# zamazincode/cv-diffusion-model

Measured on AMD Instinct MI355X. Metric: images/sec (whole node), 256×256 4-step LCM 'small'; PSNR vs CPU ref, higher is better.
Workload: dtype fp16; 1 GPU; variant=small, 256x256, batch=32/GPU, 4 LCM steps, fp16, 1xMI355X (BASELINE configs[1] per GPU); global_batch=32, parallelism=single GPU

## Files before the change

cv-diffusion-model_amd/_native.py:

```python
from __future__ import annotations

import ctypes as C
import os
from typing import List, Tuple

_HERE = os.path.dirname(os.path.abspath(__file__))
LIB_PATH = os.path.join(_HERE, "libllie_hip.so")

LLIE_F32, LLIE_F16, LLIE_BF16 = 0, 1, 2
LLIE_UNET, LLIE_IRB, LLIE_ATTN, LLIE_DOWN, LLIE_UP, LLIE_SE = 0, 1, 2, 3, 4, 5
ERR_ARG, ERR_SHAPE, ERR_CONFIG, ERR_KEY, ERR_NOT_LOADED, ERR_WORKSPACE, ERR_NO_DEVICE = -1, -2, -3, -4, -5, -6, -7

EXPORTS = [
    "llie_last_error", "llie_version", "llie_create", "llie_destroy", "llie_num_params", "llie_param_info",
    "llie_load_param", "llie_params_loaded", "llie_workspace_bytes", "llie_unet_forward", "llie_module_forward",
    "llie_lcm_step", "llie_add_noise", "llie_enhance", "llie_algorithmic_bytes", "llie_flops",
    "llie_profile_begin", "llie_profile_end", "llie_enhance_workspace_bytes",
    "llie_preprocess_u8", "llie_postprocess_u8", "llie_profile_report", "llie_pw_gemm", "llie_pw_gemm_tile_rows", "llie_dwconv3x3", "llie_dwconv3x3_tiles", "llie_tune",
    "llie_grad_numel", "llie_param_grad_offset", "llie_train_workspace_bytes", "llie_unet_train_forward",
    "llie_unet_backward", "llie_module_backward", "llie_load_all", "llie_profile_dump", "llie_copy_probe", "llie_rw_probe", "llie_pw_expand", "llie_gram_stats", "llie_gram_part_floats", "llie_groupnorm_finalize", "llie_conv3x3", "llie_conv3x3_tiles", "llie_linattn", "llie_linattn_splits", "llie_se_mlp", "llie_film", "llie_refresh_params", "llie_path_bytes", "llie_time_embed", "llie_debug_irbx_stamps", "llie_debug_gemm_stamps", "llie_debug_pwx_stamps", "llie_graph_cache_entries", "llie_debug_conv_stamps", "llie_gram_finalize",
    "llie_optimizer_create", "llie_optimizer_destroy", "llie_optimizer_numel", "llie_optimizer_step",
    "llie_optimizer_step_amp",
    "llie_consistency_target", "llie_consistency_loss", "llie_ema_create", "llie_ema_update", "llie_ema_destroy",
    "llie_wgrad", "llie_wgrad_msplit", "llie_wgrad_partial_floats", "llie_dw_wgrad", "llie_dw_wgrad_strips",
    "llie_groupnorm_backward", "llie_groupnorm_backward_scratch_floats", "llie_linattn_backward", "llie_linattn_dkv_floats",
    "llie_upsample2x_backward", "llie_dilate2x", "llie_linear_dx", "llie_linear_dx_scratch_floats", "llie_linear_dw",
    "llie_final_bwd_data",
    "llie_dwconv3x3_backward", "llie_groupnorm_backward_from_slab", "llie_bias_grad", "llie_bias_grad_floats", "llie_pack_planes",
    "llie_add_into", "llie_sin_embed", "llie_pointwise_backward",
    "llie_tile_count", "llie_tile_origins", "llie_tile_gather_u8", "llie_tile_gather_f32", "llie_tile_blend_u8",
    "llie_aug_pair_u8", "llie_aug_synth_u8",
    "llie_image_metrics_scratch_bytes", "llie_image_metrics_f32", "llie_image_metrics_u8", "llie_comparison_grid_u8",
    "llie_upconv_fold_elems", "llie_upconv_fold_weights", "llie_conv3x3_upfold", "llie_conv3x3_upfold_tiles",
    "llie_expand_dw", "llie_expand_pool", "llie_expand_dw_project", "llie_expand_dw_project_skip", "llie_irbx_project_tiles",
    "llie_expand_stats", "llie_irbx_stats_rows",
    "llie_dwconv3x3_ex", "llie_dwconv3x3_strip_rows", "llie_last_kernel",
    "llie_init_conv", "llie_init_conv_tiles", "llie_init_conv_pack_bytes", "llie_final_conv", "llie_final_conv_pack_bytes",
    "llie_se_gate", "llie_affine_add", "llie_nchw_to_nhwc", "llie_nhwc_to_nchw", "llie_pw_gemm_dot",
    "llie_frame_shape_ok", "llie_frame_workspace_bytes", "llie_unet_forward_hw", "llie_enhance_hw",
    "llie_frame_pad", "llie_frame_load_u8", "llie_frame_store_u8",
]
K_GEMM, K_DW, K_CONV3, K_SE, K_OTHER = 1, 2, 4, 8, 16
PW_SIGMOID_BWD, PW_RELU6_BWD, PW_SILU_BWD, PW_SCALE = 0, 1, 2, 3


class GemmSeg(C.Structure):
    _fields_ = [("ptr", C.c_void_p), ("channels", C.c_int), ("scale", C.c_void_p), ("bias", C.c_void_p),
                ("affine_ld", C.c_int), ("act", C.c_int)]


# ... 143 lines not shown
    L.llie_init_conv_pack_bytes.restype = i64
    L.llie_init_conv_tiles.argtypes = [ci, ci, ci]
    L.llie_init_conv.argtypes = [ci, vp, ci, vp, ci, vp, vp, vp, vp, ci, ci, ci, ci, ci, vp, i64, vp]
    L.llie_final_conv_pack_bytes.argtypes = [ci]
    L.llie_final_conv_pack_bytes.restype = i64
    L.llie_final_conv.argtypes = [ci, vp, vp, vp, vp, vp, vp, ci, ci, ci, ci, ci, ci, C.POINTER(StepCoef), vp, vp, vp, vp, vp, i64, vp]
    L.llie_se_gate.argtypes = [ci, vp, ci, vp, vp, vp, vp, vp, ci, ci, ci, ci, vp, vp, vp]
    L.llie_affine_add.argtypes = [ci, vp, vp, vp, vp, vp, vp, ci, ci, ci, vp]
    L.llie_nchw_to_nhwc.argtypes = [ci, vp, vp, vp, ci, ci, ci, ci, ci, vp]
    L.llie_nhwc_to_nchw.argtypes = [ci, vp, vp, ci, ci, ci, ci, ci, vp]
    L.llie_pw_gemm_dot.argtypes = [ci, C.POINTER(GemmSeg), ci, vp, vp, vp, vp, vp, ci, ci, ci, vp]
    L.llie_last_kernel.argtypes = []
    L.llie_last_kernel.restype = C.c_char_p
    L.llie_expand_dw.argtypes = [ci, vp, ci, vp, ci, vp, vp, vp, vp, vp, vp, vp, vp, ci, ci, ci, vp]
    L.llie_expand_pool.argtypes = [ci, vp, ci, vp, ci, vp, vp, vp, vp, vp, vp, vp, ci, ci, ci, vp]
    L.llie_expand_dw_project.argtypes = [ci, vp, ci, vp, vp, vp, vp, vp, vp, vp, vp, vp, vp, ci, ci, ci, vp]
    L.llie_expand_dw_project_skip.argtypes = [ci, vp, ci, vp, ci, vp, vp, vp, vp, vp, vp, vp, vp, ci, ci, vp, vp, ci, ci, ci, vp]
    L.llie_irbx_project_tiles.argtypes = [ci, ci]
    L.llie_expand_stats.argtypes = [ci, vp, ci, vp, ci, vp, vp, vp, vp, ci, ci, ci, vp]
    L.llie_irbx_stats_rows.argtypes = [ci]
    L.llie_tune.argtypes = [C.c_char_p, ci]
    L.llie_debug_irbx_stamps.argtypes = [C.POINTER(C.c_double)]
    L.llie_optimizer_create.argtypes = [C.POINTER(OptTensor), ci, C.POINTER(C.c_void_p)]
    L.llie_optimizer_destroy.argtypes = [C.c_void_p]
    L.llie_optimizer_destroy.restype = None
    L.llie_optimizer_numel.argtypes = [C.c_void_p]
    L.llie_optimizer_numel.restype = C.c_int64
    L.llie_optimizer_step.argtypes = [C.c_void_p, vp, C.POINTER(OptHyper), vp, vp]
    L.llie_optimizer_step_amp.argtypes = [C.c_void_p, vp, C.POINTER(OptHyper), C.POINTER(AmpState), C.POINTER(AmpConfig), vp, vp]
    L.llie_consistency_target.argtypes = [vp, vp, vp, vp, vp, ci, vp, ci, i64, vp]
# ... 192 lines not shown
```

cv-diffusion-model_amd/csrc/common.h:

```cpp
#pragma once
#include <hip/hip_runtime.h>
#include <stdint.h>

#include <atomic>
#include <type_traits>

#include "kernels.h"

namespace llie {

typedef _Float16 half_t;
typedef __bf16 bf16_t;

typedef float f32x4 __attribute__((ext_vector_type(4)));
typedef float f32x16 __attribute__((ext_vector_type(16)));
typedef _Float16 f16x8 __attribute__((ext_vector_type(8)));
typedef _Float16 f16x2 __attribute__((ext_vector_type(2)));
typedef __bf16 bf16x8 __attribute__((ext_vector_type(8)));
typedef uint32_t u32x4 __attribute__((ext_vector_type(4)));
typedef f32x4 f32x4u __attribute__((aligned(4)));

constexpr int kWave = 64;

__device__ __forceinline__ void load12(const uint8_t* s, uint32_t (&b)[12]) {
// ... 117 lines not shown
  if constexpr (std::is_same<T, half_t>::value) {
    uint32_t r;
    if constexpr (CLAMP) {
      asm("v_fma_mixlo_f16 %0, %1, %2, %3 op_sel:[0,0,0] op_sel_hi:[1,0,0] clamp" : "=v"(r) : "v"(x2), "v"(s0), "v"(b0));
      asm("v_fma_mixhi_f16 %0, %1, %2, %3 op_sel:[1,0,0] op_sel_hi:[1,0,0] clamp" : "+v"(r) : "v"(x2), "v"(s1), "v"(b1));
    } else {
      asm("v_fma_mixlo_f16 %0, %1, %2, %3 op_sel:[0,0,0] op_sel_hi:[1,0,0]" : "=v"(r) : "v"(x2), "v"(s0), "v"(b0));
      asm("v_fma_mixhi_f16 %0, %1, %2, %3 op_sel:[1,0,0] op_sel_hi:[1,0,0]" : "+v"(r) : "v"(x2), "v"(s1), "v"(b1));
    }
    return r;
  } else {
    return affine_clamp01_pack<T, CLAMP>(__uint_as_float(x2 << 16), __uint_as_float(x2 & 0xFFFF0000u), s0, s1, b0, b1);
  }
}

__device__ __forceinline__ float wave_sum(float v) {
#pragma unroll
  for (int o = 32; o > 0; o >>= 1) v += __shfl_xor(v, o, 64);
  return v;
}
__device__ __forceinline__ double wave_sum(double v) {
#pragma unroll
  for (int o = 32; o > 0; o >>= 1) v += __shfl_xor(v, o, 64);
  return v;
}

constexpr int kPoolSegRows = 8;
template <int VEC>
__device__ __forceinline__ void pool_segment_flush(float (&psum)[VEC], float* red_wave , int lane) {
  static_assert(VEC == 8 || VEC == 4, "");
// ... 89 lines not shown
```

cv-diffusion-model_amd/csrc/engine.h:

```cpp
#pragma once
#include <hip/hip_runtime.h>

#include <algorithm>
#include <cmath>
#include <cstdarg>
#include <cstdio>
#include <cstdlib>
#include <cstring>
#include <map>
#include <tuple>
#include <string>
#include <vector>

#include "../../include/llie.h"
#include "kernels.h"

namespace llie {

void set_err(const char* fmt, ...);
inline hipStream_t hs(llie_stream stream) { return reinterpret_cast<hipStream_t>(stream); }

inline size_t elem_size(int dt) { return dt == LLIE_F32 ? 4 : 2; }
inline size_t align_up(size_t x, size_t a) { return (x + a - 1) / a * a; }

// ... 178 lines not shown
    if (hipEventCreate(&e) != hipSuccess) return nullptr;
    return e;
  }
};

namespace llie {

struct Knobs {
  int use_irbx;
  int irbx_project;
  int gram;
  int nt_min_mb;
  int nt_mask;
  int se_mfma;
  int bwd_async;
  int upconv_fold;
  int enhance_split;
  int epoch;
};
extern Knobs g_knobs;

enum IrbForm { kIrbUnfused, kIrbRecompute, kIrbProject };
struct IrbPath {
  IrbForm form;
  bool s6;
  bool fixtot;
  bool gram;
};
inline IrbPath irb_path(int dt, const IrbW& w, int c0, int H, int W, bool training) {
  IrbPath p{kIrbUnfused, !training && dt != LLIE_F32, !training && w.hid % 128 == 0, false};
  if (!p.fixtot || !g_knobs.use_irbx || w.hid != w.hid_r || w.cin != w.cin_r || !irbx_supported(dt, w.cin, c0, w.hid, H, W)) return p;
  p.gram = g_knobs.gram && (H * W >= 32768 || g_knobs.gram > 1) && gram_supported(dt, w.cin, c0, H * W);
  const int tail = g_knobs.irbx_project && w.cout == w.cout_r ? irbx_project_supported(dt, w.cin, c0, w.hid, w.cout, w.skip, H, W) : 0;
  p.form = tail && !(tail == kIrbxProjectSkip && g_knobs.irbx_project == 2) ? kIrbProject : kIrbRecompute;
  return p;
}

inline bool upconv_fold_supported(int dt, int Hi, int Wi, int C) {
  return g_knobs.upconv_fold && (C == 64 || C == 128) && conv3x3_upfold_ok(dt, Hi, Wi, C);
}

struct Exec {
  llie_ctx* c;
  Arena* ar;
  hipStream_t s;
// ... 40 lines not shown
```

cv-diffusion-model_amd/csrc/forward.cpp:

```cpp
#include "engine.h"

using namespace llie;

namespace {

struct Run : Exec {
  Tape* tape = nullptr;
  char tag[56] = "";
  void rel(size_t off) { if (!tape) ar->free(off); }
  size_t zoff = 0, zcur = 0, zcap = 0;
  bool zcount = false;
  template <typename F> void zbegin(int H, int W, F&& forward_again) {
    if (tape || zcount) return;
    const auto key = std::make_tuple(B, H, W, g_knobs.epoch);
    auto it = c->zneed.find(key);
    if (it == c->zneed.end()) {
      size_t zbytes = 0;
      plan(c, B, forward_again, &zbytes);
      it = c->zneed.emplace(key, zbytes).first;
    }
    zcap = it->second;
    if (!zcap) return;
    zoff = ar->alloc(zcap);
    if (!dry) chk(launch_zero_fill(ws + zoff, (int64_t)zcap, s));
// ... 115 lines not shown
    gn(h1, nullptr, w.n2g, w.n2b, film, film_stride, t.as2, t.ab2, &rec.n2, path.s6 ? 1.f / 6.f : 0.f);
    t.dnt = dwconv_ntiles(H, W);
    t.h2 = ar->alloc((size_t)M * w.hid * es());
    t.pool = path.fixtot ? 0 : ar->alloc((size_t)B * t.dnt * w.hid * 4);
    t.ptot = path.fixtot ? ztake((size_t)B * w.hid * 8) : 0;
    if (!dry) {
      DwArgs d{};
      d.in = p(h1.off); d.out = p(t.h2); d.as = p<float>(t.as2); d.ab = p<float>(t.ab2); d.w = wptr<float>(w.w_dw);
      if (path.fixtot) d.pool_tot = p<unsigned long long>(t.ptot); else d.pool = p<float>(t.pool);
      d.B = B; d.H = H; d.W = W; d.C = w.hid; d.s6 = path.s6 ? 1 : 0; d.nt = nt_store(4, (int64_t)M * w.hid);
      timed(LLIE_K_DW, 2LL * M * w.hid * (int64_t)es(), [&] { return launch_dwconv3x3(dt, d, s); });
    }
    rel(t.as1); rel(t.ab1); rel(h1.off); rel(h1.slab); rel(t.as2); rel(t.ab2);
  }

  IrbxArgs irbx_args(const IrbW& w, const Tens& x0, const Tens* x1, size_t as1, size_t ab1) const {
    IrbxArgs a{};
    a.x0 = p(x0.off); a.c0 = x0.C; a.x1 = x1 ? p(x1->off) : nullptr; a.c1 = x1 ? x1->C : 0; a.as1 = p<float>(as1); a.ab1 = p<float>(ab1);
    a.w1 = wptr(w.w_expand); a.wd = wptr<float>(w.w_dw); a.B = B; a.H = x0.H; a.W = x0.W; a.Chid = w.hid;
    return a;
  }
  void front_recompute(const IrbPath& path, const IrbW& w, const Tens& x0, const Tens* x1, const float* film, int64_t film_stride, IrbTmp& t) {
    const int H = x0.H, W = x0.W, P = H * W, M = B * P;
    const bool pool_only = path.form == kIrbProject;
    Tens st;
    st.C = w.hid; st.Cr = w.hid_r; st.H = H; st.W = W; st.ntiles = P / irbx_stats_rows(P); st.valid = true;
    st.slab = path.gram ? 0 : ar->alloc((size_t)B * st.ntiles * 2 * w.hid * 4);
    const size_t gpart = path.gram ? ar->alloc((size_t)B * gram_part_floats(w.cin, P) * 4) : 0;
    const size_t gtot = path.gram ? ar->alloc((size_t)B * (w.cin * w.cin + w.cin) * 4) : 0;
    const size_t gtick = path.gram ? ztake((size_t)B * 4) : 0;
// ... 96 lines not shown
            [&] { return launch_expand_dw_project(dt, a, w.cout, w.skip, s); });
    }
    rel(t.as1); rel(t.ab1); rel(t.as2); rel(t.ab2); rel(t.gate);
    return y;
  }

  Tens irb(const IrbW& w, const Tens& x0, const Tens* x1, const float* film, int64_t film_stride) {
    const int P = x0.H * x0.W;
    const IrbPath path = irb_path(dt, w, x0.C, x0.H, x0.W, tape != nullptr);
    IrbRec rec{};
    IrbTmp t;
    snprintf(tag, sizeof tag, "irb P=%d %d->%d hid=%d", P, w.cin, w.cout, w.hid);
    gn(x0, x1, w.n1g, w.n1b, nullptr, 0, t.as1, t.ab1, &rec.n1, path.s6 ? 1.f / 6.f : 0.f);
    const float* film2 = film ? film + w.film_off : nullptr;
    if (path.form == kIrbUnfused) front_unfused(path, w, x0, x1, film2, film_stride, rec, t);
    else front_recompute(path, w, x0, x1, film2, film_stride, t);
    se_gate(path, w, P, t);
    Tens y = path.form == kIrbProject ? project_fused(w, x0, t) : project_gemm(w, x0, x1, t);
    if (tape) {
      rec.w = (int)(&w - c->irbs.data());
      rec.x0 = x0; rec.cat = x1 != nullptr;
      if (x1) rec.x1 = *x1;
      rec.h1 = t.h1; rec.h2 = t.h2; rec.gate = t.gate; rec.sehid = t.sehid; rec.semean = t.semean; rec.y = y;
      tape->ops.push_back({0, (int)tape->irbs.size()});
      tape->irbs.push_back(rec);
    }
    return y;
  }

  Tens attn(const AttnW& w, const Tens& x) {
// ... 339 lines not shown
```

cv-diffusion-model_amd/csrc/irbx.hip:

```cpp
#include <string>
#include <type_traits>
#include <vector>

#include "common.h"
#include "kernels.h"

namespace llie {

typedef uint32_t u32x2 __attribute__((ext_vector_type(2)));

typedef __bf16 bf16x2_t __attribute__((ext_vector_type(2)));
__device__ __forceinline__ float dot2_bf16(uint32_t a, uint32_t b, float c) {
  return __builtin_amdgcn_fdot2_f32_bf16(*reinterpret_cast<const bf16x2_t*>(&a), *reinterpret_cast<const bf16x2_t*>(&b), c, false);
}

template <typename T>
__device__ __forceinline__ typename Elem<T>::vec_t activate8(typename Elem<T>::vec_t v, const float* sc, const float* sh) {
  const u32x4 x = reinterpret_cast<const u32x4&>(v);
  const f32x4 s0 = *reinterpret_cast<const f32x4*>(sc), s1 = *reinterpret_cast<const f32x4*>(sc + 4);
  const f32x4 b0 = *reinterpret_cast<const f32x4*>(sh), b1 = *reinterpret_cast<const f32x4*>(sh + 4);
  u32x4 o;
  o[0] = act_clamp01_pack<T>(x[0], s0[0], s0[1], b0[0], b0[1]);
  o[1] = act_clamp01_pack<T>(x[1], s0[2], s0[3], b0[2], b0[3]);
  o[2] = act_clamp01_pack<T>(x[2], s1[0], s1[1], b1[0], b1[1]);
  o[3] = act_clamp01_pack<T>(x[3], s1[2], s1[3], b1[2], b1[3]);
  return reinterpret_cast<const typename Elem<T>::vec_t&>(o);
}

constexpr int kXStamps = 9;
template <typename T> struct PackedOne;
template <> struct PackedOne<half_t> { static constexpr uint32_t lo = 0x00003C00u, hi = 0x3C000000u; };
template <> struct PackedOne<bf16_t> { static constexpr uint32_t lo = 0x00003F80u, hi = 0x3F800000u; };
template <typename T> __device__ __forceinline__ float dot2_pk(uint32_t a, uint32_t b, float c) {
  if constexpr (std::is_same<T, half_t>::value)
    return __builtin_amdgcn_fdot2(*reinterpret_cast<const f16x2*>(&a), *reinterpret_cast<const f16x2*>(&b), c, false);
  else return dot2_bf16(a, b, c);
}

template <typename T, int KS, int NBW, bool POOL, bool STAMP = false>
__device__ __forceinline__ void expand_scan(const IrbxArgs& a, const int RP) {
  constexpr int K = 16 * KS, XP = (K + 8) * 2;
// ... 938 lines not shown
```

cv-diffusion-model_amd/csrc/kernel_api.cpp:

```cpp
#include "engine.h"

using namespace llie;

static bool dtype_ok(int dtype) { return dtype >= 0 && dtype <= 2; }

int llie::kerr(const char* what, hipError_t e, int refuse_rc, const char* refuse_msg) {
  if (e == hipSuccess) return LLIE_OK;
  if (e == hipErrorInvalidValue && refuse_rc) {
    if (refuse_msg) set_err("%s: %s", what, refuse_msg);
    return refuse_rc;
  }
  set_err("%s: %s", what, hipGetErrorString(e));
  return (int)e;
}

static int to_segs(const llie_gemm_seg* segs, int nseg, GemmSeg* out) {
  int K = 0;
  for (int i = 0; i < nseg; ++i) {
    out[i] = GemmSeg{segs[i].ptr, segs[i].channels, segs[i].scale, segs[i].bias, segs[i].affine_ld, segs[i].act};
    K += segs[i].channels;
  }
  return K;
}

// ... 740 lines not shown
  a.gate = gate; a.wp = w_project; a.y = y; a.ystats = stats;
  return kerr("expand_dw_project", launch_expand_dw_project(dtype, a, C, false, hs(stream)), LLIE_ERR_SHAPE,
              "2-byte dtype, C in {32, 64}, H % 8 == 0, W % 16 == 0");
}
int llie_expand_dw_project_skip(int dtype, const void* x0, int c0, const void* x1, int c1, const float* scale1, const float* shift1,
                                const void* w_expand, const float* scale2, const float* shift2, const float* w_dw, const float* gate,
                                const void* w_project_skip, int ld, int cout, void* y, float* stats, int batch, int H, int W, llie_stream stream) {
  if (!x0 || !scale1 || !shift1 || !w_expand || !scale2 || !shift2 || !w_dw || !gate || !w_project_skip || !y || !stats || batch <= 0 || c0 <= 0 ||
      c1 < 0 || (c1 > 0) != (x1 != nullptr) || cout <= 0 || ld < 5 * (c0 + c1))
    return LLIE_ERR_ARG;
  IrbxArgs a = irbx_args(x0, c0, x1, c1, scale1, shift1, w_expand, scale2, shift2, w_dw, batch, H, W);
  a.gate = gate; a.wp = w_project_skip; a.ldp = ld; a.y = y; a.ystats = stats;
  return kerr("expand_dw_project_skip", launch_expand_dw_project(dtype, a, cout, true, hs(stream)), LLIE_ERR_SHAPE,
              "2-byte dtype, c0 + c1 == 96, c0 % 16 == 0, cout == 32, ld % 8 == 0, H % 8 == 0, W % 16 == 0");
}
int llie_irbx_project_tiles(int H, int W) { return H > 0 && W > 0 && H % 8 == 0 && W % 16 == 0 ? irbx_project_tiles(H, W) : LLIE_ERR_ARG; }

int llie_dwconv3x3_tiles(int H, int W) { return dwconv_ntiles(H, W); }
int llie_pw_gemm_tile_rows(int P) { return pw_gemm_tile_rows(P); }
}
```

cv-diffusion-model_amd/csrc/kernels.h:

```cpp
#pragma once
#include <hip/hip_runtime.h>
#include <stdint.h>

namespace llie {

enum Act : int { ACT_NONE = 0, ACT_RELU6 = 1, ACT_SILU = 2, ACT_RELU6_S6 = 3 };

void note_kernel(const char* name);
const char* last_kernel();

struct StatSrc {
  const float* slab;
  int ntiles;
  int ch;
};

struct GemmSeg {
  const void* ptr;
  int ch;
  const float* as;
  const float* ab;
  int aff_ld;
  int act;
};
// ... 118 lines not shown
};
void irbx_grid(int ks, int v);
void irbx_stamp(int v);
hipError_t irbx_stamp_fetch(double* out10);
bool irbx_supported(int dtype, int Cin, int c0, int Chid, int H, int W);
int irbx_pool_tiles(int H, int W);
constexpr int kIrbxProjectIdentity = 1, kIrbxProjectSkip = 2;
int irbx_project_supported(int dtype, int Cin, int c0, int Chid, int Cout, bool skip, int H, int W);
int irbx_project_tiles(int H, int W);
int irbx_stats_rows(int P);
void irbx_tune(int dbuf);
hipError_t launch_expand_stats(int dtype, const IrbxArgs& a, hipStream_t s);
hipError_t launch_expand_dw(int dtype, const IrbxArgs& a, hipStream_t s);
hipError_t launch_expand_pool(int dtype, const IrbxArgs& a, hipStream_t s);
hipError_t launch_expand_dw_project(int dtype, const IrbxArgs& a, int cout, bool skip, hipStream_t s);
int dwconv_ntiles(int H, int W);
int dw_pick_tyl(int B, int H, int W, int chunks);

struct SeArgs {
  const float* pool; int ntiles; int P;
  int pool_stride;
  const void* w1; const float* b1;
  const void* w2; const float* b2;
  float* mean;
  float* hid;
  float* gate;
  int B, C, Cs;
  const unsigned long long* tot;
  long long* pre;
};
// ... 330 lines not shown
```

cv-diffusion-model_amd/csrc/tune.cpp:

```cpp
#include "engine.h"

using namespace llie;

static Knobs knob_defaults() {
  Knobs k{};
  k.use_irbx = getenv("LLIE_NO_IRBX") ? 0 : 1;
  k.irbx_project = 1;
  k.gram = 1;
  k.nt_min_mb = 100; k.nt_mask = 1;
  k.upconv_fold = 1;
  k.se_mfma = 1;
  k.bwd_async = 1;
  k.enhance_split = getenv("LLIE_ENHANCE_SPLIT") ? atoi(getenv("LLIE_ENHANCE_SPLIT")) : 2;
  k.epoch = 0;
  return k;
}
Knobs llie::g_knobs = knob_defaults();

static hipError_t elapsed_ms(const llie_ctx::ProfRec& r, float* ms) {
  hipError_t e = hipEventSynchronize(r.e1);
  if (e == hipSuccess) e = hipEventElapsedTime(ms, r.e0, r.e1);
  if (e != hipSuccess) set_err("profile: %s", hipGetErrorString(e));
  return e;
}

// ... 2 lines not shown
  hipError_t e = hipDeviceSynchronize();
  if (e == hipSuccess) e = fetch(out);
  return e == hipSuccess ? LLIE_OK : LLIE_ERR_ARG;
}

extern "C" {

int llie_tune(const char* knob, int value) {
  if (!knob) return LLIE_ERR_ARG;
  ++g_knobs.epoch;
  if (!strcmp(knob, "gemm_bk")) { pw_gemm_force_bk(value); return LLIE_OK; }
  if (!strcmp(knob, "se_mfma")) { g_knobs.se_mfma = value; return LLIE_OK; }
  if (!strcmp(knob, "nt_min_mb")) { g_knobs.nt_min_mb = value; return LLIE_OK; }
  if (!strcmp(knob, "nt_mask")) { g_knobs.nt_mask = value; return LLIE_OK; }
  if (!strcmp(knob, "upconv_fold")) { g_knobs.upconv_fold = value != 0; return LLIE_OK; }
  if (!strcmp(knob, "gram")) { g_knobs.gram = value; return LLIE_OK; }
  if (!strcmp(knob, "irbx")) { g_knobs.use_irbx = value != 0; return LLIE_OK; }
  if (!strcmp(knob, "irbx_project")) { g_knobs.irbx_project = value < 0 || value > 2 ? 1 : value; return LLIE_OK; }
  if (!strcmp(knob, "irbx_dbuf")) { irbx_tune(value); return LLIE_OK; }
  if (!strcmp(knob, "irbx_stamp")) { irbx_stamp(value); return LLIE_OK; }
  if (!strcmp(knob, "irbx_grid")) { irbx_grid(0, value); return LLIE_OK; }
  if (!strcmp(knob, "irbx_grid2")) { irbx_grid(2, value); return LLIE_OK; }
  if (!strcmp(knob, "irbx_grid4")) { irbx_grid(4, value); return LLIE_OK; }
  if (!strcmp(knob, "irbx_grid6")) { irbx_grid(6, value); return LLIE_OK; }
  if (!strcmp(knob, "conv_stamp")) { conv3x3_stamp(value); return LLIE_OK; }
  if (!strcmp(knob, "gemm_stamp")) { pw_gemm_stamp(value); return LLIE_OK; }
  if (!strcmp(knob, "pwx")) { pw_expand_enable(value); return LLIE_OK; }
  if (!strcmp(knob, "pwx_stamp")) { pw_expand_debug(value); return LLIE_OK; }
  if (!strcmp(knob, "bwd_async")) { g_knobs.bwd_async = value; return LLIE_OK; }
  if (!strcmp(knob, "enhance_split")) { g_knobs.enhance_split = value; return LLIE_OK; }
// ... 73 lines not shown
```

include/llie.h:

```cpp
#ifndef LLIE_H_
#define LLIE_H_

#include <stddef.h>
#include <stdint.h>

#ifdef __cplusplus
extern "C" {
#endif

typedef struct llie_ctx llie_ctx;
typedef void* llie_stream;

enum llie_status {
  LLIE_OK = 0,
  LLIE_ERR_ARG = -1,
  LLIE_ERR_SHAPE = -2,
  LLIE_ERR_CONFIG = -3,
  LLIE_ERR_KEY = -4,
  LLIE_ERR_NOT_LOADED = -5,
  LLIE_ERR_WORKSPACE = -6,
  LLIE_ERR_NO_DEVICE = -7
};

enum llie_dtype { LLIE_F32 = 0, LLIE_F16 = 1, LLIE_BF16 = 2 };
// ... 271 lines not shown
                   const float* scale2, const float* shift2, const float* w_dw, void* h2, unsigned long long* pool_totals, int batch, int H, int W,
                   llie_stream stream);
int llie_expand_pool(int dtype, const void* x0, int c0, const void* x1, int c1, const float* scale1, const float* shift1, const void* w_expand,
                     const float* scale2, const float* shift2, const float* w_dw, unsigned long long* pool_totals, int batch, int H, int W,
                     llie_stream stream);
int llie_expand_dw_project(int dtype, const void* x, int C, const float* scale1, const float* shift1, const void* w_expand, const float* scale2,
                           const float* shift2, const float* w_dw, const float* gate, const void* w_project, void* y, float* stats, int batch,
                           int H, int W, llie_stream stream);
int llie_expand_dw_project_skip(int dtype, const void* x0, int c0, const void* x1, int c1, const float* scale1, const float* shift1,
                                const void* w_expand, const float* scale2, const float* shift2, const float* w_dw, const float* gate,
                                const void* w_project_skip, int ld, int cout, void* y, float* stats, int batch, int H, int W, llie_stream stream);
int llie_irbx_project_tiles(int H, int W);
int llie_expand_stats(int dtype, const void* x0, int c0, const void* x1, int c1, const float* scale1, const float* shift1, const void* w_expand,
                      float* stats, int batch, int H, int W, llie_stream stream);
int llie_irbx_stats_rows(int P);
int llie_copy_probe(const void* src, void* dst, int64_t bytes, llie_stream stream);
int llie_rw_probe(const void* src, void* dst, int64_t units, int reads, int writes, int nontemporal, llie_stream stream);
int llie_tune(const char* knob, int value);
int llie_debug_irbx_stamps(double* out10);
int llie_debug_conv_stamps(double* out8);
int llie_debug_gemm_stamps(double* out3);
int llie_debug_pwx_stamps(double* out4);

enum llie_kernel_class {
  LLIE_K_GEMM = 1,
  LLIE_K_DW = 2,
  LLIE_K_CONV3 = 4,
  LLIE_K_SE = 8,
  LLIE_K_OTHER = 16
};
// ... 17 lines not shown
```

Baseline: 1207 images/sec.

## Add fused expand+groupnorm+dwconv kernel holding the whole 32x32 map in LDS

Adds a new IRB front-end kernel for 1024-pixel maps (32x32) with 128 input channels. One workgroup keeps a 64-channel slab of the expanded activations for a whole image in LDS. It runs the expand GEMM with MFMA, computes GroupNorm statistics in place, applies norm+FiLM+ReLU6, then the 3x3 depthwise conv, and writes pooled SE sums, all without writing the intermediate to HBM or launching a separate stats pass. The path is enabled by default through a knob. The cost is one workgroup per CU from about 141KB of LDS, and it applies only to low-resolution layers.

Result: no change. 1205 images/sec (-0.2%).

```diff
diff --git a/cv-diffusion-model_amd/_native.py b/cv-diffusion-model_amd/_native.py
--- a/cv-diffusion-model_amd/_native.py
+++ b/cv-diffusion-model_amd/_native.py
@@ -33,7 +33,7 @@
     "llie_image_metrics_scratch_bytes", "llie_image_metrics_f32", "llie_image_metrics_u8", "llie_comparison_grid_u8",
     "llie_upconv_fold_elems", "llie_upconv_fold_weights", "llie_conv3x3_upfold", "llie_conv3x3_upfold_tiles",
     "llie_expand_dw", "llie_expand_pool", "llie_expand_dw_project", "llie_expand_dw_project_skip", "llie_irbx_project_tiles",
-    "llie_expand_stats", "llie_irbx_stats_rows",
+    "llie_expand_stats", "llie_irbx_stats_rows", "llie_expand_dw_map", "llie_irb_map_supported",
     "llie_dwconv3x3_ex", "llie_dwconv3x3_strip_rows", "llie_last_kernel",
     "llie_init_conv", "llie_init_conv_tiles", "llie_init_conv_pack_bytes", "llie_final_conv", "llie_final_conv_pack_bytes",
     "llie_se_gate", "llie_affine_add", "llie_nchw_to_nhwc", "llie_nhwc_to_nchw", "llie_pw_gemm_dot",
@@ -207,6 +207,8 @@
     L.llie_last_kernel.restype = C.c_char_p
     L.llie_expand_dw.argtypes = [ci, vp, ci, vp, ci, vp, vp, vp, vp, vp, vp, vp, vp, ci, ci, ci, vp]
     L.llie_expand_pool.argtypes = [ci, vp, ci, vp, ci, vp, vp, vp, vp, vp, vp, vp, ci, ci, ci, vp]
+    L.llie_expand_dw_map.argtypes = [ci, vp, ci, vp, ci, vp, vp, vp, vp, vp, vp, vp, i64, C.c_float, vp, vp, vp, ci, ci, ci, vp]
+    L.llie_irb_map_supported.argtypes = [ci, ci, ci, ci, ci]
     L.llie_expand_dw_project.argtypes = [ci, vp, ci, vp, vp, vp, vp, vp, vp, vp, vp, vp, vp, ci, ci, ci, vp]
     L.llie_expand_dw_project_skip.argtypes = [ci, vp, ci, vp, ci, vp, vp, vp, vp, vp, vp, vp, vp, ci, ci, vp, vp, ci, ci, ci, vp]
     L.llie_irbx_project_tiles.argtypes = [ci, ci]
diff --git a/cv-diffusion-model_amd/csrc/common.h b/cv-diffusion-model_amd/csrc/common.h
--- a/cv-diffusion-model_amd/csrc/common.h
+++ b/cv-diffusion-model_amd/csrc/common.h
@@ -155,6 +155,19 @@
   }
 }
 
+template <typename T>
+__device__ __forceinline__ typename Elem<T>::vec_t activate8(typename Elem<T>::vec_t v, const float* sc, const float* sh) {
+  const u32x4 x = reinterpret_cast<const u32x4&>(v);
+  const f32x4 s0 = *reinterpret_cast<const f32x4*>(sc), s1 = *reinterpret_cast<const f32x4*>(sc + 4);
+  const f32x4 b0 = *reinterpret_cast<const f32x4*>(sh), b1 = *reinterpret_cast<const f32x4*>(sh + 4);
+  u32x4 o;
+  o[0] = act_clamp01_pack<T>(x[0], s0[0], s0[1], b0[0], b0[1]);
+  o[1] = act_clamp01_pack<T>(x[1], s0[2], s0[3], b0[2], b0[3]);
+  o[2] = act_clamp01_pack<T>(x[2], s1[0], s1[1], b1[0], b1[1]);
+  o[3] = act_clamp01_pack<T>(x[3], s1[2], s1[3], b1[2], b1[3]);
+  return reinterpret_cast<const typename Elem<T>::vec_t&>(o);
+}
+
 __device__ __forceinline__ float wave_sum(float v) {
 #pragma unroll
   for (int o = 32; o > 0; o >>= 1) v += __shfl_xor(v, o, 64);
diff --git a/cv-diffusion-model_amd/csrc/engine.h b/cv-diffusion-model_amd/csrc/engine.h
--- a/cv-diffusion-model_amd/csrc/engine.h
+++ b/cv-diffusion-model_amd/csrc/engine.h
@@ -216,13 +216,14 @@
   int nt_mask;
   int se_mfma;
   int bwd_async;
+  int irb_map;
   int upconv_fold;
   int enhance_split;
   int epoch;
 };
 extern Knobs g_knobs;
 
-enum IrbForm { kIrbUnfused, kIrbRecompute, kIrbProject };
+enum IrbForm { kIrbUnfused, kIrbRecompute, kIrbProject, kIrbMap };
 struct IrbPath {
   IrbForm form;
   bool s6;
@@ -231,6 +232,10 @@
 };
 inline IrbPath irb_path(int dt, const IrbW& w, int c0, int H, int W, bool training) {
   IrbPath p{kIrbUnfused, !training && dt != LLIE_F32, !training && w.hid % 128 == 0, false};
+  if (p.fixtot && p.s6 && g_knobs.irb_map && w.cin == 128 && w.has_wf && w.hid == w.hid_r && w.cin == w.cin_r && irb_map_supported(dt, w.cin, c0, w.hid, H, W)) {
+    p.form = kIrbMap;
+    return p;
+  }
   if (!p.fixtot || !g_knobs.use_irbx || w.hid != w.hid_r || w.cin != w.cin_r || !irbx_supported(dt, w.cin, c0, w.hid, H, W)) return p;
   p.gram = g_knobs.gram && (H * W >= 32768 || g_knobs.gram > 1) && gram_supported(dt, w.cin, c0, H * W);
   const int tail = g_knobs.irbx_project && w.cout == w.cout_r ? irbx_project_supported(dt, w.cin, c0, w.hid, w.cout, w.skip, H, W) : 0;
diff --git a/cv-diffusion-model_amd/csrc/forward.cpp b/cv-diffusion-model_amd/csrc/forward.cpp
--- a/cv-diffusion-model_amd/csrc/forward.cpp
+++ b/cv-diffusion-model_amd/csrc/forward.cpp
@@ -153,6 +153,22 @@
     rel(t.as1); rel(t.ab1); rel(h1.off); rel(h1.slab); rel(t.as2); rel(t.ab2);
   }
 
+  void front_map(const IrbW& w, const Tens& x0, const Tens* x1, const float* film, int64_t film_stride, IrbTmp& t) {
+    const int H = x0.H, W = x0.W, P = H * W, M = B * P;
+    t.dnt = dwconv_ntiles(H, W);
+    t.h2 = ar->alloc((size_t)M * w.hid * es());
+    t.ptot = ztake((size_t)B * w.hid * 8);
+    if (!dry) {
+      IrbMapArgs a{};
+      a.x0 = p(x0.off); a.c0 = x0.C; a.x1 = x1 ? p(x1->off) : nullptr; a.c1 = x1 ? x1->C : 0; a.as1 = p<float>(t.as1); a.ab1 = p<float>(t.ab1);
+      a.wf = wptr(w.w_expand_f); a.gamma = wptr<float>(w.n2g); a.beta = wptr<float>(w.n2b); a.film = film; a.film_stride = film_stride;
+      a.eps = 1e-5f; a.wd = wptr<float>(w.w_dw); a.out = p(t.h2); a.pool_tot = p<unsigned long long>(t.ptot);
+      a.B = B; a.H = H; a.W = W; a.Chid = w.hid;
+      timed(LLIE_K_DW, ((int64_t)M * (w.cin + w.hid) + (int64_t)w.hid * w.cin) * (int64_t)es(), [&] { return launch_expand_dw_map(dt, a, s); });
+    }
+    rel(t.as1); rel(t.ab1);
+  }
+
   IrbxArgs irbx_args(const IrbW& w, const Tens& x0, const Tens* x1, size_t as1, size_t ab1) const {
     IrbxArgs a{};
     a.x0 = p(x0.off); a.c0 = x0.C; a.x1 = x1 ? p(x1->off) : nullptr; a.c1 = x1 ? x1->C : 0; a.as1 = p<float>(as1); a.ab1 = p<float>(ab1);
@@ -279,6 +295,7 @@
     gn(x0, x1, w.n1g, w.n1b, nullptr, 0, t.as1, t.ab1, &rec.n1, path.s6 ? 1.f / 6.f : 0.f);
     const float* film2 = film ? film + w.film_off : nullptr;
     if (path.form == kIrbUnfused) front_unfused(path, w, x0, x1, film2, film_stride, rec, t);
+    else if (path.form == kIrbMap) front_map(w, x0, x1, film2, film_stride, t);
     else front_recompute(path, w, x0, x1, film2, film_stride, t);
     se_gate(path, w, P, t);
     Tens y = path.form == kIrbProject ? project_fused(w, x0, t) : project_gemm(w, x0, x1, t);
diff --git a/cv-diffusion-model_amd/csrc/irbm.hip b/cv-diffusion-model_amd/csrc/irbm.hip
--- /dev/null
+++ b/cv-diffusion-model_amd/csrc/irbm.hip
@@ -0,0 +1,284 @@
+#include <string>
+#include <type_traits>
+
+#include "common.h"
+#include "kernels.h"
+
+namespace llie {
+
+typedef uint32_t u32x2m __attribute__((ext_vector_type(2)));
+
+constexpr int kMapP = 1024;
+constexpr int kMapNT = 512;
+constexpr int kMapKmax = 512;
+constexpr int kLdsPerCU = 163840;
+
+template <int CW> constexpr size_t irb_map_lds_bytes() {
+  return (size_t)kMapP * CW * 2 + 2 * kMapKmax * 4 + 2 * CW * 4 + 9 * CW * 4 + 8 * (CW / 8) * 2 * 8 + 8 * CW * 4;
+}
+static_assert(irb_map_lds_bytes<64>() == 141056 && irb_map_lds_bytes<64>() <= kLdsPerCU, "expand_dw_map<64>: one workgroup per CU");
+
+template <typename T> __device__ __forceinline__ uint32_t pack2(float a, float b) {
+  typedef T t2 __attribute__((ext_vector_type(2)));
+  t2 o;
+  o[0] = (T)a; o[1] = (T)b;
+  return *reinterpret_cast<uint32_t*>(&o);
+}
+
+template <typename T, int CW>
+__global__ void __launch_bounds__(kMapNT, 1) expand_dw_map_kernel(const IrbMapArgs a) {
+  static_assert(CW == 64, "a 64-channel chunk: eight 16-byte slots per pixel");
+  typedef typename Elem<T>::vec_t vec_t;
+  extern __shared__ __align__(16) unsigned char smem[];
+  unsigned char* map = smem;
+  float* aff1 = reinterpret_cast<float*>(smem + (size_t)kMapP * CW * 2);
+  float* aff2 = aff1 + 2 * kMapKmax;
+  float* wds = aff2 + 2 * CW;
+  double* sred = reinterpret_cast<double*>(wds + 9 * CW);
+  float* pred = reinterpret_cast<float*>(sred + 8 * (CW / 8) * 2);
+
+  const int tid = threadIdx.x, lane = tid & 63, wave = tid >> 6;
+  const int n = lane & 31, h = lane >> 5;
+  const int nch = a.Chid / CW;
+  const int v = xcd_tile_order((int)(blockIdx.z * gridDim.x + blockIdx.x), (int)(gridDim.x * gridDim.z));
+  const int b = v / nch, chunk = v - b * nch;
+  const int K = a.c0 + a.c1, KS = K / 16;
+  auto slot_ptr = [&](int p, int s) { return map + p * (CW * 2) + ((s ^ ((p >> 1) & 7)) << 4); };
+
+  for (int i = tid; i < K; i += kMapNT) {
+    aff1[i] = a.as1[(size_t)b * K + i];
+    aff1[kMapKmax + i] = a.ab1[(size_t)b * K + i];
+  }
+  for (int i = tid; i < 9 * CW; i += kMapNT) wds[i] = (float)(T)(6.f * a.wd[(i / CW) * a.Chid + chunk * CW + (i % CW)]);
+  wg_barrier();
+
+  {
+    const T* x0 = reinterpret_cast<const T*>(a.x0) + (size_t)b * kMapP * a.c0;
+    const T* x1 = a.x1 ? reinterpret_cast<const T*>(a.x1) + (size_t)b * kMapP * a.c1 : nullptr;
+    const T* wf = reinterpret_cast<const T*>(a.wf) + (size_t)chunk * (CW / 32) * KS * 512 + lane * 8;
+    const int p0 = wave * 128 + n;
+    f32x16 acc[4][2];
+#pragma unroll
+    for (int i = 0; i < 4; ++i)
+#pragma unroll
+      for (int cb = 0; cb < 2; ++cb)
+#pragma unroll
+        for (int r = 0; r < 16; ++r) acc[i][cb][r] = 0.f;
+    auto load_x = [&](int ss, vec_t (&xr)[2][4]) {
+      const bool seg1 = 32 * ss >= a.c0;
+      const int cs = seg1 ? a.c1 : a.c0;
+      const T* base = (seg1 ? x1 - a.c0 : x0) + 32 * ss + 8 * h;
+#pragma unroll
+      for (int j = 0; j < 2; ++j)
+#pragma unroll
+        for (int i = 0; i < 4; ++i) xr[j][i] = ld_vec<T>(base + 16 * j + (size_t)(p0 + 32 * i) * cs);
+    };
+    auto load_w = [&](int s, vec_t (&wr)[2]) {
+#pragma unroll
+      for (int cb = 0; cb < 2; ++cb) wr[cb] = ld_vec<T>(wf + (size_t)(cb * KS + s) * 512);
+    };
+    auto compute = [&](int s, const vec_t (&xr)[4], const vec_t (&wr)[2]) {
+      const int k = 16 * s + 8 * h;
+#pragma unroll
+      for (int i = 0; i < 4; ++i) {
+        const vec_t av = activate8<T>(xr[i], aff1 + k, aff1 + kMapKmax + k);
+#pragma unroll
+        for (int cb = 0; cb < 2; ++cb) acc[i][cb] = mfma16<T>(wr[cb], av, acc[i][cb]);
+      }
+    };
+    vec_t xa[2][4], xb[2][4], w0[2], w1[2];
+    load_w(0, w0);
+    load_x(0, xa);
+    for (int s = 0; s < KS; s += 4) {
+      load_w(s + 1, w1);
+      load_x(s / 2 + 1, xb);
+      compute(s, xa[0], w0);
+      load_w(s + 2, w0);
+      compute(s + 1, xa[1], w1);
+      load_w(s + 3, w1);
+      if (s + 4 < KS) load_x(s / 2 + 2, xa);
+      compute(s + 2, xb[0], w0);
+      if (s + 4 < KS) load_w(s + 4, w0);
+      compute(s + 3, xb[1], w1);
+    }
+#pragma unroll
+    for (int i = 0; i < 4; ++i) {
+      const int p = p0 + 32 * i;
+#pragma unroll
+      for (int cb = 0; cb < 2; ++cb) {
+        const f32x16 ac = acc[i][cb];
+        uint32_t pk[4][2];
+#pragma unroll
+        for (int g = 0; g < 4; ++g)
+#pragma unroll
+          for (int j = 0; j < 2; ++j) pk[g][j] = pack2<T>(ac[4 * g + 2 * j], ac[4 * g + 2 * j + 1]);
+        u32x4 lo, hi2;
+#pragma unroll
+        for (int j = 0; j < 2; ++j) {
+          const u32x2m r02 = __builtin_amdgcn_permlane32_swap(pk[0][j], pk[2][j], false, false);
+          const u32x2m r13 = __builtin_amdgcn_permlane32_swap(pk[1][j], pk[3][j], false, false);
+          lo[j] = r02[0]; lo[2 + j] = r02[1];
+          hi2[j] = r13[0]; hi2[2 + j] = r13[1];
+        }
+        *reinterpret_cast<u32x4*>(slot_ptr(p, cb * 4 + 2 * h)) = lo;
+        *reinterpret_cast<u32x4*>(slot_ptr(p, cb * 4 + 2 * h + 1)) = hi2;
+      }
+    }
+  }
+  wg_barrier();
+
+  const int slot = tid & 7, col = tid >> 3;
+  {
+    float s1 = 0.f, s2 = 0.f;
+#pragma unroll 4
+    for (int i = 0; i < kMapP / 64; ++i) {
+      const vec_t hv = *reinterpret_cast<const vec_t*>(slot_ptr(col + 64 * i, slot));
+#pragma unroll
+      for (int e = 0; e < 8; ++e) {
+        const float f = (float)hv[e];
+        s1 += f;
+        s2 = __builtin_fmaf(f, f, s2);
+      }
+    }
+    double d1 = (double)s1, d2 = (double)s2;
+#pragma unroll
+    for (int o = 8; o < 64; o <<= 1) {
+      d1 += __shfl_xor(d1, o, 64);
+      d2 += __shfl_xor(d2, o, 64);
+    }
+    if (lane < 8) {
+      sred[(wave * 8 + lane) * 2] = d1;
+      sred[(wave * 8 + lane) * 2 + 1] = d2;
+    }
+    wg_barrier();
+    if (tid < CW) {
+      const int cg = a.Chid / 32, c = chunk * CW + tid;
+      const int sl0 = (tid / cg) * (cg / 8), sl1 = sl0 + cg / 8;
+      double t1 = 0.0, t2 = 0.0;
+      for (int sl = sl0; sl < sl1; ++sl)
+#pragma unroll
+        for (int w = 0; w < 8; ++w) {
+          t1 += sred[(w * 8 + sl) * 2];
+          t2 += sred[(w * 8 + sl) * 2 + 1];
+        }
+      const double cnt = (double)cg * (double)kMapP;
+      const double mean = t1 / cnt;
+      double var = t2 / cnt - mean * mean;
+      if (var < 0.0) var = 0.0;
+      const float rstd = (float)(1.0 / sqrt(var + (double)a.eps));
+      const float fmean = (float)mean;
+      const float ga = a.gamma[c] * rstd;
+      float sc = ga, sh = a.beta[c] - fmean * ga;
+      if (a.film) {
+        const float* f = a.film + (size_t)b * a.film_stride;
+        const float fs = 1.f + f[c], fh = f[a.Chid + c];
+        sc *= fs;
+        sh = sh * fs + fh;
+      }
+      aff2[tid] = sc * kSixth;
+      aff2[CW + tid] = sh * kSixth;
+    }
+    wg_barrier();
+#pragma unroll 4
+    for (int i = 0; i < kMapP / 64; ++i) {
+      vec_t* hp = reinterpret_cast<vec_t*>(slot_ptr(col + 64 * i, slot));
+      *hp = activate8<T>(*hp, aff2 + 8 * slot, aff2 + CW + 8 * slot);
+    }
+    wg_barrier();
+  }
+
+  f32x2 wv[9][4];
+#pragma unroll
+  for (int t = 0; t < 9; ++t)
+#pragma unroll
+    for (int q = 0; q < 4; ++q) wv[t][q] = *reinterpret_cast<const f32x2*>(wds + t * CW + 8 * slot + 2 * q);
+  f32x2 ps[4] = {{0.f, 0.f}, {0.f, 0.f}, {0.f, 0.f}, {0.f, 0.f}};
+  T* out = reinterpret_cast<T*>(a.out) + (size_t)b * kMapP * a.Chid + chunk * CW + 8 * slot;
+  const int W = a.W, H = a.H;
+  auto walk = [&](auto nr_c, int unit) {
+    constexpr int NR = decltype(nr_c)::value;
+    const int band = unit / W, x = unit - band * W, y0 = band * NR;
+    const bool okl = x > 0, okr = x + 1 < W;
+    f32x2 win[3][3][4];
+#pragma unroll
+    for (int r = 0; r < NR + 2; ++r) {
+      const int yi = y0 + r - 1;
+      const bool rowok = yi >= 0 && yi < H;
+#pragma unroll
+      for (int dx = 0; dx < 3; ++dx) {
+        const bool ok = rowok && (dx == 0 ? okl : dx == 2 ? okr : true);
+        const int p = ok ? yi * W + x + dx - 1 : 0;
+        const vec_t hv = *reinterpret_cast<const vec_t*>(slot_ptr(p, slot));
+#pragma unroll
+        for (int q = 0; q < 4; ++q) win[r % 3][dx][q] = ok ? f32x2{(float)hv[2 * q], (float)hv[2 * q + 1]} : f32x2{0.f, 0.f};
+      }
+      if (r >= 2) {
+        f32x2 o[4] = {{0.f, 0.f}, {0.f, 0.f}, {0.f, 0.f}, {0.f, 0.f}};
+#pragma unroll
+        for (int ky = 0; ky < 3; ++ky)
+#pragma unroll
+          for (int kx = 0; kx < 3; ++kx)
+#pragma unroll
+            for (int q = 0; q < 4; ++q) o[q] = __builtin_elementwise_fma(win[(r - 2 + ky) % 3][kx][q], wv[ky * 3 + kx][q], o[q]);
+        u32x4 st;
+#pragma unroll
+        for (int q = 0; q < 4; ++q) {
+          ps[q] += o[q];
+          st[q] = pack2<T>(o[q][0], o[q][1]);
+        }
+        *reinterpret_cast<u32x4*>(out + (size_t)((y0 + r - 2) * W + x) * a.Chid) = st;
+      }
+    }
+  };
+  if (H >= 16) {
+    walk(std::integral_constant<int, 16>{}, col);
+  } else {
+    walk(std::integral_constant<int, 8>{}, col);
+    walk(std::integral_constant<int, 8>{}, col + 64);
+  }
+  float pv[8];
+#pragma unroll
+  for (int q = 0; q < 4; ++q) { pv[2 * q] = ps[q][0]; pv[2 * q + 1] = ps[q][1]; }
+#pragma unroll
+  for (int e = 0; e < 8; ++e)
+#pragma unroll
+    for (int o = 8; o < 64; o <<= 1) pv[e] += __shfl_xor(pv[e], o, 64);
+  if (lane < 8) {
+#pragma unroll
+    for (int e = 0; e < 8; ++e) pred[wave * CW + 8 * lane + e] = pv[e];
+  }
+  wg_barrier();
+  if (tid < CW) {
+    float t = 0.f;
+#pragma unroll
+    for (int w = 0; w < 8; ++w) t += pred[w * CW + tid];
+    a.pool_tot[(size_t)b * a.Chid + chunk * CW + tid] = (unsigned long long)__float2ll_rn(t * kPoolFixScale);
+  }
+}
+
+bool irb_map_supported(int dtype, int Cin, int c0, int Chid, int H, int W) {
+  if (dtype != 1 && dtype != 2) return false;
+  if (Cin != 128 && Cin != 256 && Cin != 512) return false;
+  if (Chid != 4 * Cin || c0 <= 0 || c0 > Cin || c0 % 64 || (Cin - c0) % 64) return false;
+  return H > 0 && W > 0 && H % 8 == 0 && W % 16 == 0 && (long long)H * W == kMapP;
+}
+
+template <typename T>
+static hipError_t launch_map_t(const IrbMapArgs& a, hipStream_t s) {
+  constexpr int CW = 64;
+  constexpr size_t lds = irb_map_lds_bytes<CW>();
+  static const std::string name = std::string("expand_dw_map_kernel<") + TypeName<T>::value + ", " + std::to_string(CW) + ">";
+  note_kernel(name.c_str());
+  static std::atomic<uint64_t> attr_done{0};
+  if (hipError_t e = ensure_max_lds(reinterpret_cast<const void*>(&expand_dw_map_kernel<T, CW>), (int)lds, attr_done); e != hipSuccess) return e;
+  hipLaunchKernelGGL((expand_dw_map_kernel<T, CW>), dim3(a.Chid / CW, 1, a.B), dim3(kMapNT), lds, s, a);
+  return hipGetLastError();
+}
+hipError_t launch_expand_dw_map(int dtype, const IrbMapArgs& a, hipStream_t s) {
+  if (!irb_map_supported(dtype, a.c0 + a.c1, a.c0, a.Chid, a.H, a.W) || (a.c1 != 0) != (a.x1 != nullptr) || a.B <= 0 || a.B > 65535 || !a.x0 ||
+      !a.as1 || !a.ab1 || !a.wf || !a.gamma || !a.beta || !a.wd || !a.out || !a.pool_tot)
+    return hipErrorInvalidValue;
+  return dtype == 1 ? launch_map_t<half_t>(a, s) : launch_map_t<bf16_t>(a, s);
+}
+
+}
diff --git a/cv-diffusion-model_amd/csrc/irbx.hip b/cv-diffusion-model_amd/csrc/irbx.hip
--- a/cv-diffusion-model_amd/csrc/irbx.hip
+++ b/cv-diffusion-model_amd/csrc/irbx.hip
@@ -12,19 +12,6 @@
 typedef __bf16 bf16x2_t __attribute__((ext_vector_type(2)));
 __device__ __forceinline__ float dot2_bf16(uint32_t a, uint32_t b, float c) {
   return __builtin_amdgcn_fdot2_f32_bf16(*reinterpret_cast<const bf16x2_t*>(&a), *reinterpret_cast<const bf16x2_t*>(&b), c, false);
-}
-
-template <typename T>
-__device__ __forceinline__ typename Elem<T>::vec_t activate8(typename Elem<T>::vec_t v, const float* sc, const float* sh) {
-  const u32x4 x = reinterpret_cast<const u32x4&>(v);
-  const f32x4 s0 = *reinterpret_cast<const f32x4*>(sc), s1 = *reinterpret_cast<const f32x4*>(sc + 4);
-  const f32x4 b0 = *reinterpret_cast<const f32x4*>(sh), b1 = *reinterpret_cast<const f32x4*>(sh + 4);
-  u32x4 o;
-  o[0] = act_clamp01_pack<T>(x[0], s0[0], s0[1], b0[0], b0[1]);
-  o[1] = act_clamp01_pack<T>(x[1], s0[2], s0[3], b0[2], b0[3]);
-  o[2] = act_clamp01_pack<T>(x[2], s1[0], s1[1], b1[0], b1[1]);
-  o[3] = act_clamp01_pack<T>(x[3], s1[2], s1[3], b1[2], b1[3]);
-  return reinterpret_cast<const typename Elem<T>::vec_t&>(o);
 }
 
 constexpr int kXStamps = 9;
diff --git a/cv-diffusion-model_amd/csrc/kernel_api.cpp b/cv-diffusion-model_amd/csrc/kernel_api.cpp
--- a/cv-diffusion-model_amd/csrc/kernel_api.cpp
+++ b/cv-diffusion-model_amd/csrc/kernel_api.cpp
@@ -778,6 +778,24 @@
   return kerr("expand_dw_project_skip", launch_expand_dw_project(dtype, a, cout, true, hs(stream)), LLIE_ERR_SHAPE,
               "2-byte dtype, c0 + c1 == 96, c0 % 16 == 0, cout == 32, ld % 8 == 0, H % 8 == 0, W % 16 == 0");
 }
+static const char* kIrbMapShapes = "2-byte dtype, c0 + c1 in {128, 256, 512}, c0 and c1 multiples of 64, H % 8 == 0, W % 16 == 0, H * W == 1024";
+int llie_irb_map_supported(int dtype, int Cin, int c0, int H, int W) { return irb_map_supported(dtype, Cin, c0, 4 * Cin, H, W) ? 1 : 0; }
+int llie_expand_dw_map(int dtype, const void* x0, int c0, const void* x1, int c1, const float* scale1, const float* shift1, const float* w32,
+                       void* wpack, const float* gamma2, const float* beta2, const float* film, int64_t film_stride, float eps,
+                       const float* w_dw, void* h2, unsigned long long* pool_totals, int batch, int H, int W, llie_stream stream) {
+  if (!x0 || !scale1 || !shift1 || !wpack || !gamma2 || !beta2 || !w_dw || !h2 || !pool_totals || batch <= 0 || c0 <= 0 || c1 < 0 ||
+      (c1 > 0) != (x1 != nullptr))
+    return LLIE_ERR_ARG;
+  IrbMapArgs a{};
+  a.x0 = x0; a.c0 = c0; a.x1 = x1; a.c1 = c1; a.as1 = scale1; a.ab1 = shift1; a.wf = wpack; a.gamma = gamma2; a.beta = beta2;
+  a.film = film; a.film_stride = film_stride; a.eps = eps; a.wd = w_dw; a.out = h2; a.pool_tot = pool_totals;
+  a.B = batch; a.H = H; a.W = W; a.Chid = 4 * (c0 + c1);
+  hipStream_t s = hs(stream);
+  hipError_t e = !irb_map_supported(dtype, c0 + c1, c0, a.Chid, H, W) ? hipErrorInvalidValue
+                 : (w32 ? launch_pack_expand(dtype, w32, wpack, a.Chid, c0 + c1, 6.f, s) : hipSuccess);
+  if (e == hipSuccess) e = launch_expand_dw_map(dtype, a, s);
+  return kerr("expand_dw_map", e, LLIE_ERR_SHAPE, kIrbMapShapes);
+}
 int llie_irbx_project_tiles(int H, int W) { return H > 0 && W > 0 && H % 8 == 0 && W % 16 == 0 ? irbx_project_tiles(H, W) : LLIE_ERR_ARG; }
 
 int llie_dwconv3x3_tiles(int H, int W) { return dwconv_ntiles(H, W); }
diff --git a/cv-diffusion-model_amd/csrc/kernels.h b/cv-diffusion-model_amd/csrc/kernels.h
--- a/cv-diffusion-model_amd/csrc/kernels.h
+++ b/cv-diffusion-model_amd/csrc/kernels.h
@@ -156,6 +156,20 @@
 hipError_t launch_expand_dw(int dtype, const IrbxArgs& a, hipStream_t s);
 hipError_t launch_expand_pool(int dtype, const IrbxArgs& a, hipStream_t s);
 hipError_t launch_expand_dw_project(int dtype, const IrbxArgs& a, int cout, bool skip, hipStream_t s);
+struct IrbMapArgs {
+  const void* x0; const void* x1; int c0, c1;
+  const float* as1; const float* ab1;
+  const void* wf;
+  const float* gamma; const float* beta;
+  const float* film; int64_t film_stride;
+  float eps;
+  const float* wd;
+  void* out;
+  unsigned long long* pool_tot;
+  int B, H, W, Chid;
+};
+bool irb_map_supported(int dtype, int Cin, int c0, int Chid, int H, int W);
+hipError_t launch_expand_dw_map(int dtype, const IrbMapArgs& a, hipStream_t s);
 int dwconv_ntiles(int H, int W);
 int dw_pick_tyl(int B, int H, int W, int chunks);
 
diff --git a/cv-diffusion-model_amd/csrc/tune.cpp b/cv-diffusion-model_amd/csrc/tune.cpp
--- a/cv-diffusion-model_amd/csrc/tune.cpp
+++ b/cv-diffusion-model_amd/csrc/tune.cpp
@@ -9,6 +9,7 @@
   k.gram = 1;
   k.nt_min_mb = 100; k.nt_mask = 1;
   k.upconv_fold = 1;
+  k.irb_map = getenv("LLIE_NO_IRB_MAP") ? 0 : 1;
   k.se_mfma = 1;
   k.bwd_async = 1;
   k.enhance_split = getenv("LLIE_ENHANCE_SPLIT") ? atoi(getenv("LLIE_ENHANCE_SPLIT")) : 2;
@@ -41,6 +42,7 @@
   if (!strcmp(knob, "nt_min_mb")) { g_knobs.nt_min_mb = value; return LLIE_OK; }
   if (!strcmp(knob, "nt_mask")) { g_knobs.nt_mask = value; return LLIE_OK; }
   if (!strcmp(knob, "upconv_fold")) { g_knobs.upconv_fold = value != 0; return LLIE_OK; }
+  if (!strcmp(knob, "irb_map")) { g_knobs.irb_map = value != 0; return LLIE_OK; }
   if (!strcmp(knob, "gram")) { g_knobs.gram = value; return LLIE_OK; }
   if (!strcmp(knob, "irbx")) { g_knobs.use_irbx = value != 0; return LLIE_OK; }
   if (!strcmp(knob, "irbx_project")) { g_knobs.irbx_project = value < 0 || value > 2 ? 1 : value; return LLIE_OK; }
diff --git a/include/llie.h b/include/llie.h
--- a/include/llie.h
+++ b/include/llie.h
@@ -309,6 +309,10 @@
 int llie_expand_stats(int dtype, const void* x0, int c0, const void* x1, int c1, const float* scale1, const float* shift1, const void* w_expand,
                       float* stats, int batch, int H, int W, llie_stream stream);
 int llie_irbx_stats_rows(int P);
+int llie_irb_map_supported(int dtype, int Cin, int c0, int H, int W);
+int llie_expand_dw_map(int dtype, const void* x0, int c0, const void* x1, int c1, const float* scale1, const float* shift1, const float* w32,
+                       void* wpack, const float* gamma2, const float* beta2, const float* film, int64_t film_stride, float eps,
+                       const float* w_dw, void* h2, unsigned long long* pool_totals, int batch, int H, int W, llie_stream stream);
 int llie_copy_probe(const void* src, void* dst, int64_t bytes, llie_stream stream);
 int llie_rw_probe(const void* src, void* dst, int64_t units, int reads, int writes, int nontemporal, llie_stream stream);
 int llie_tune(const char* knob, int value);
```
